# electronicarts/mesh2splat

Hardware: AMD Instinct MI355X
Metric: Gaussians/sec emitted (mesh->3DGS conversion pass, density 1024^2) (higher is better)
Workload: dtype f32

## Files before the change

mesh2splat_amd/csrc/m2s_context.cpp:

```cpp
#include "m2s_ctx.h"

#include <algorithm>
#include <chrono>
#include <cstring>
#include <string>

using namespace m2s;
using namespace m2s_host;

namespace {
thread_local std::string g_create_error = "";
}

namespace m2s_host {
void free_scene(m2s_ctx* c) {
    c->tri_mem.release(); c->scene_arena.release();
    c->lane[0].release_scene(false); c->lane[1].release_scene(true);
    c->d_meshes = nullptr; c->d_mesh_first = nullptr;
    c->d_cnt = c->d_partials = nullptr;
    c->d_biglist = nullptr; c->d_bigmeta = nullptr; c->d_bands = nullptr; c->run_table_words = 0; c->d_run_order = nullptr; c->run_order_unit = 0;
    c->d_batch_first = nullptr; c->n_batch_tab = 0; c->chain_words = 0;
    c->rinfo.clear();
    ++c->rinfo_gen;
    c->frag_per_R2 = -1.0;
    c->warm_R = 0; c->warm_total = 0; c->warm_mismatch_seen = false;
    c->sparse_off_R = c->team_off_R = c->lean_off_R = UINT32_MAX;
    c->lean_ok = false;
    c->d_vt_rows.release(); c->d_vt_ids.release();
    c->vt_rows = 0; c->vt_use = false;
    c->geo_stride = 0; c->geo_use = false;
    c->scene = SceneDev{};
    c->has_scene = false;
}

m2s_ctx::RInfo& rinfo_for(m2s_ctx* c, uint32_t R) {
    auto it = c->rinfo.find(R);
    if (it != c->rinfo.end()) return it->second;
    if (c->rinfo.size() >= (size_t)kBandSlots) { drain_in_flight(c); c->rinfo.clear(); ++c->rinfo_gen; }
    m2s_ctx::RInfo ri;
    ri.gen = c->rinfo_gen;
    ri.band_slot = (int)c->rinfo.size();
    return c->rinfo.emplace(R, ri).first->second;
}

static bool spin_waits() { static const bool on = !debug_on("M2S_NO_SPIN"); return on; }
template <class Query, class Block>
static hipError_t spin_then_block(Query query, Block block) {
    if (spin_waits()) {
        const auto t0 = std::chrono::steady_clock::now();
        for (uint32_t i = 0;; ++i) {
            const hipError_t e = query();
            if (e != hipErrorNotReady) return e;
            if ((i & 15u) == 15u && std::chrono::steady_clock::now() - t0 > std::chrono::microseconds(400)) break;
        }
        (void)hipGetLastError();
    }
    return block();
}
hipError_t wait_stream(hipStream_t st) { return spin_then_block([&] { return hipStreamQuery(st); }, [&] { return hipStreamSynchronize(st); }); }
hipError_t wait_event(hipEvent_t ev) { return spin_then_block([&] { return hipEventQuery(ev); }, [&] { return hipEventSynchronize(ev); }); }

void drain_in_flight(m2s_ctx* c, int lane) {
    each_in_flight(c, [&](m2s_ctx::Slot& sl) {
        if (!sl.sync_result && (lane < 0 || sl.own_lane == lane)) (void)hipEventSynchronize(sl.done[0]);
    });
}

hipError_t next_epoch(m2s_ctx* c, uint32_t* out) {
    const uint32_t e = ++c->epoch;
    *out = e;
    if ((e & 0xFFFFu) != 0) return hipSuccess;
    const size_t bytes = std::max<size_t>(c->chain_words, 1) * sizeof(unsigned long long);
    hipError_t r = hipDeviceSynchronize();
// ... 160 lines not shown
```

mesh2splat_amd/csrc/m2s_ctx.h:

```cpp
#pragma once
#include "../../include/m2s.h"
#include "m2s_devbuf.h"
#include "m2s_device.h"
#include "m2s_recstate.h"
#include "m2s_vdedup.h"

#include <cstdint>
#include <cstdlib>
#include <map>
#include <string>

namespace m2s_host {
constexpr uint32_t kMaxGaussiansToSort = 7000000u;
constexpr uint64_t kMaxTriangles = (1ull << 28) - 1;
inline size_t align_up(size_t v, size_t a) { return (v + a - 1) / a * a; }
inline const char* const kStaleMsg = "the records of the conversion last waited for have been overwritten by a later submission at another R "
                                     "(wait for it, or submit into your own buffers)";
inline const char* const kInFlightMsg = "conversions are still in flight: m2s_convert_wait first";
struct GBufPlanes {
    DevBuf<void> plane[5];
    void* ptr[5] = {};
    m2s_status reserve(std::string& err, uint64_t px) {
        for (int k = 0; k < 5; ++k) {
            const m2s_status s = plane[k].reserve(err, px, (k == 2 || k == 4) ? 4 : 8);
// ... 5 lines not shown
};
}

constexpr int kBandSlotsMax = 64;
struct m2s_ctx : m2s_host::RecordState {
    int device = 0;
    m2s_host::StreamSet<2> streams;
    hipStream_t stream = nullptr;
    std::string err;

    m2s_host::DevBuf<char> tri_mem;
    m2s::SceneDev scene{};
    m2s::MeshParams* d_meshes = nullptr;
    uint32_t* d_mesh_first = nullptr;
    uint32_t n_meshes_total = 0;
    bool has_scene = false;
    bool lean_ok = false;
    uint64_t range_first = 0, range_count = UINT64_MAX;
    m2s_host::DevBuf<float4> d_vt_rows;
    m2s_host::DevBuf<m2s::VtIds> d_vt_ids;
    uint32_t vt_rows = 0;
    bool vt_use = false;
    m2s_host::DevBuf<float4> d_geo;
    size_t geo_stride = 0;
    bool geo_use = false;

    uint32_t* d_cnt = nullptr;
    uint32_t* d_partials = nullptr;
    m2s_host::PinnedBuf<unsigned long long> h_total;
    static constexpr int kPinnedPrepass = 2 + 2 * M2S_MAX_IN_FLIGHT;
    static constexpr int kPinnedSortMM = 4 + 2 * M2S_MAX_IN_FLIGHT;
    static constexpr int kPinnedWords = 6 + 2 * M2S_MAX_IN_FLIGHT;
    m2s::BigItem* d_biglist = nullptr;
    uint32_t* d_bigmeta = nullptr;
    struct RInfo {
        int form = M2S_PIPELINE_AUTO;
        uint32_t tpw = 0;
        bool async_ok = false;
        bool mp_ready = false;
        bool bands_ready = false;
        uint32_t bands_unit = 0;
        int band_slot = 0;
        uint32_t gen = 0;
    };
    uint32_t sparse_off_R = UINT32_MAX, team_off_R = UINT32_MAX, lean_off_R = UINT32_MAX;
    uint32_t rinfo_gen = 0;
    std::map<uint32_t, RInfo> rinfo;
    double frag_per_R2 = -1.0;
    uint64_t warm_total = 0;
    uint64_t warm_big = 0;
    bool warm_mismatch_seen = false;
    uint32_t hint_R = 0;
    uint32_t warm_R = 0;
    int warm_spec_form = 0;
    uint32_t warm_spec_unit = 0, warm_spec_shift = 0;
    unsigned long long* d_bands = nullptr;
    size_t run_table_words = 0;
    uint32_t* d_run_order = nullptr;
    uint32_t run_order_unit = 0, run_order_shift = 0;
    uint32_t* d_batch_first = nullptr;
    uint32_t n_batch_tab = 0;
    size_t chain_words = 0;
    int last_pipeline = 0;
    m2s_host::Lane lane[2];
    int lanes = 1;
    int pipeline = M2S_PIPELINE_AUTO;
    uint32_t epoch = 0;

    struct Slot { m2s_host::EventSet<1> done; m2s_host::EventSet<2> t;
                  uint64_t limit = 0; void* d_out = nullptr; uint32_t R = 0;
                  bool sync_result = false; uint64_t sync_total = 0; bool prof = false; float ms[M2S_K_N] = {};
                  int own_lane = -1; uint32_t gen = 0;
                  bool wrote_bands = false; uint32_t bands_unit = 0; uint32_t ri_gen = 0;
                  hipStream_t st = nullptr; bool shared_work = false; };
    Slot slot[M2S_MAX_IN_FLIGHT];
    uint32_t slot_head = 0, slot_count = 0;

    int64_t cap_policy = -1;

    m2s_host::DevBuf<float4> d_sorted;
    m2s_host::DevBuf<uint32_t> d_sort_u32;
    uint32_t sorted_key_offset = 0;
    m2s_host::DevBuf<void> d_sort_temp;
    float last_sort_ms = 0.0f;
    float last_sort_stage_ms[3] = { 0, 0, 0 };
    m2s_host::ClockOf<m2s_host::SortMark> sort_clock;
    m2s_host::DevBuf<float4> d_pos_plane;
    bool keep_positions = false;
    m2s_host::DevBuf<float4> d_quads;
    m2s_host::DevBuf<float> d_pp_depths;
    m2s_host::DevBuf<unsigned long long> d_pp_chain;
    uint32_t pp_epoch = 0;
    m2s_host::DevBuf<float> d_pp_depthtex;
    float last_prepass_ms = 0.0f;
    m2s_host::ClockOf<m2s_host::SpanMark> prepass_clock;
    m2s_host::PinnedBuf<m2s_gaussian> h_export[2];
    m2s_host::PinnedBuf<char> h_stage[2];
    m2s_host::DevBuf<char> d_stage[2];
    m2s_host::EventSet<2> stage_ev;
    m2s_host::DevBuf<char> scene_arena;
    float last_upload_ms[5] = { 0, 0, 0, 0, 0 };
    m2s_host::DevBuf<uint8_t> d_rows;
    m2s_host::DevBuf<void> d_loaded;
    m2s_host::DevBuf<float4> d_sorted_quads;
    float last_sort_prepass_ms = 0.0f;
    m2s_host::ClockOf<m2s_host::SpanMark> sort_prepass_clock;
    m2s_host::GBufPlanes d_gbuf;
    int32_t gbuf_w = 0, gbuf_h = 0;
    m2s_host::BinWork splat_work;
    m2s_host::DevBuf<uint32_t> d_splat_tiles;
    float last_splat_ms = 0.0f;
    m2s_host::ClockOf<m2s_host::BinMark> bin_clock;
// ... 231 lines not shown
```

mesh2splat_amd/csrc/m2s_device.h:

```cpp
#pragma once
#include <cstdlib>
#include <hip/hip_runtime.h>
#include <stdint.h>

#include "m2s_stageclock.h"
#include "m2s_vtable.h"

namespace m2s {
using m2s_host::StageMarks;

#ifdef M2S_DEBUG_BUILD
inline const char* debug_env(const char* name) {
    static const bool enabled = std::getenv("M2S_DEBUG") != nullptr;
    return enabled ? std::getenv(name) : nullptr;
}
#else
inline const char* debug_env(const char*) { return nullptr; }
#endif
inline bool debug_on(const char* name) { const char* v = debug_env(name); return v && *v && *v != '0'; }

constexpr int kBlock = 256;
constexpr int kTriPerBlock = 1024;
constexpr int kEmitF = 1024;
constexpr int kRowsThread = 32;
// ... 10 lines not shown
    const float4* C1;
    const float*  C2;
    const float4* D0;
    const float4* D1;
    const float4* D2;
};

struct TexDesc {
    const uint32_t* texels;
    uint32_t w, h, n_levels;
    uint32_t off[5];
};

struct ComboDesc {
    const uint32_t* texels;
    uint32_t coff[5];
};

struct MeshParams {
    float bmin[3];
    float bmax[3];
    float color[4];
    TexDesc tex[3];
    ComboDesc combo;
};

struct BigItem {
    uint32_t t, cnt;
    unsigned long long off;
};

struct SceneDev {
    TriPlanes tri;
    const MeshParams* meshes;
    const uint32_t* mesh_first;
    const uint2* mesh_of8;
    uint32_t n_meshes;
    uint32_t n_tri;
    uint32_t tri_first;
};

void launch_repack(const float* d_aos, uint32_t stride_floats, uint32_t n_tri_src, uint32_t src_first,
                   uint32_t n, uint32_t dst_first, TriPlanes dst , hipStream_t st);
void launch_mesh_table(const SceneDev& sc, uint2* table, hipStream_t st);
void launch_mip_level(const uint32_t* src, uint32_t sw, uint32_t sh, uint32_t* dst, uint32_t dw, uint32_t dh,
                      hipStream_t st);
void launch_combo_level(const uint32_t* a, const uint32_t* n, const uint32_t* m, uint32_t w, uint32_t h, uint32_t* dst,
                        hipStream_t st);
void launch_count(const SceneDev& sc, uint32_t R, uint32_t* cnt, uint32_t* partials, hipStream_t st);
void launch_scan_partials(uint32_t* partials, uint32_t n_partials, unsigned long long* total, hipStream_t st);
void launch_big_share(const uint32_t* cnt, uint32_t n_tri, uint32_t threshold, unsigned long long* out, hipStream_t st);
void launch_unit_bases(const uint32_t* cnt, const uint32_t* partials, uint32_t n_tri, uint32_t unit, uint32_t shift, unsigned long long* run_base, hipStream_t st);
void launch_run_order(const unsigned long long* run_base, uint32_t n_runs, const unsigned long long* total, uint32_t* order, uint32_t n_slots,
                      uint32_t first_set, hipStream_t st);
inline uint32_t resident_workgroups(const void* kernel, int threads) {
    int dev = 0, cus = 0, per_cu = 0;
    if (hipGetDevice(&dev) != hipSuccess || hipDeviceGetAttribute(&cus, hipDeviceAttributeMultiprocessorCount, dev) != hipSuccess ||
        hipOccupancyMaxActiveBlocksPerMultiprocessor(&per_cu, kernel, threads, 0) != hipSuccess || cus <= 0 || per_cu <= 0) {
        (void)hipGetLastError();
        return 0u;
    }
    return (uint32_t)per_cu * (uint32_t)cus;
}
uint32_t fused2_resident_workgroups();
uint32_t fused3_resident_workgroups();
uint32_t sparse_resident_workgroups();
inline uint32_t run_order_slots(uint32_t n_units, uint32_t shift) { return ((n_units + (8u << shift) - 1u) / (8u << shift)) * 8u; }
uint32_t emit2_slices(uint64_t limit);
uint32_t count_scan_blocks(uint32_t n_tri);
size_t setup_bytes(uint32_t n_tri);
size_t setup_tall_offset(uint32_t n_tri);
void launch_count_scan(const SceneDev& sc, uint32_t R, uint32_t* off, uint32_t* start, uint32_t n_start, unsigned long long* chain,
                       uint32_t epoch, unsigned long long* total, void* setup, uint32_t* status, unsigned long long* total_host, hipStream_t st);
void launch_emit2(const SceneDev& sc, uint32_t R, const uint32_t* off, const uint32_t* start, const unsigned long long* total,
                  uint64_t limit, const void* setup, float4* out, hipStream_t st);

void launch_encode_rows(const float4* rec, uint64_t n, uint32_t format, float scale_multiplier, uint8_t* out, hipStream_t st);

struct RunInfo {
    const unsigned long long* base;
    unsigned long long* out;
    uint32_t shift;
    const uint32_t* order;
};
inline uint32_t run_shift_for(uint32_t n_units) {
    if (const char* v = debug_env("M2S_RUN_SHIFT")) { const uint32_t s = (uint32_t)std::atoi(v) & 15u; return n_units >= (32u << s) ? s : 0u; }
    for (uint32_t shift = 5; shift >= 3; --shift)
        if (n_units >= (32u << shift)) return shift;
    return 0u;
}
inline uint32_t n_runs(uint32_t n_units, uint32_t shift) { return (n_units + (1u << shift) - 1u) >> shift; }
struct BatchTable {
    const uint32_t* first;
    uint32_t n;
    uint32_t tpw;
};
uint32_t fused2_band_workgroups(uint32_t n_tri);
void launch_fused2(const SceneDev& sc, uint32_t R, unsigned long long* chain, uint64_t limit, float4* out,
                   unsigned long long* total, uint32_t* status, uint32_t epoch, BigItem* biglist, uint32_t* bigmeta,
                   const RunInfo& runs, const BatchTable& batches, hipStream_t st);
struct GeoPlanes {
    const float4* G0;
    const float4* G1;
    const float4* G2;
};
void launch_geo_planes(const SceneDev& sc, float4* g0, float4* g1, float4* g2, hipStream_t st);
void launch_fused3(const SceneDev& sc, uint32_t R, unsigned long long* chain, uint64_t limit, float4* out,
                   unsigned long long* total, uint32_t* status, uint32_t epoch, BigItem* biglist, uint32_t* bigmeta,
                   const RunInfo& runs, const BatchTable& batches, hipStream_t st, const VtxTable* vt = nullptr,
                   const GeoPlanes* gp = nullptr);
void launch_sparse(const SceneDev& sc, uint32_t R, unsigned long long* chain, uint64_t limit, float4* out,
                   unsigned long long* total, uint32_t* status, uint32_t epoch, BigItem* biglist, uint32_t* bigmeta,
                   const RunInfo& runs, hipStream_t st, float4* plane = nullptr);
bool sparse_supported(uint32_t n_tri);
uint32_t sparse_workgroups(uint32_t n_tri);
constexpr uint32_t kSparseTrianglesPerWorkgroup = 512;
void launch_emit_big(const SceneDev& sc, uint32_t R, const BigItem* biglist, uint32_t n_big, uint32_t max_cnt, uint64_t limit,
                     float4* out, hipStream_t st);

struct PrepassK {
// ... 233 lines not shown
```

mesh2splat_amd/csrc/m2s_kernels.hip:

```cpp
#include "m2s_devfn.h"

#pragma clang fp contract(off)

namespace m2s {

struct TriPlanesW {
    float4* A0; float4* A1; float* A2; float4* B0; float2* B1; float4* C0; float4* C1; float* C2;
    float4* D0; float4* D1; float4* D2;
};

__global__ void __launch_bounds__(kBlock) k_repack(const float* __restrict__ aos, uint32_t stride, uint32_t src_first,
                                                   uint32_t n, uint32_t dst_first, TriPlanesW d) {
    uint32_t i = blockIdx.x * kBlock + threadIdx.x;
    if (i >= n) return;
    const float* v0 = aos + (size_t)(src_first + i) * 3 * stride;
    const float* v1 = v0 + stride;
    const float* v2 = v1 + stride;
    uint32_t t = dst_first + i;
    d.A0[t] = make_float4(v0[0], v0[1], v0[2], v1[0]);
    d.A1[t] = make_float4(v1[1], v1[2], v2[0], v2[1]);
    d.A2[t] = v2[2];
    d.B0[t] = make_float4(v0[10], v0[11], v1[10], v1[11]);
    d.B1[t] = make_float2(v2[10], v2[11]);
    d.C0[t] = make_float4(v0[3], v0[4], v0[5], v1[3]);
    d.C1[t] = make_float4(v1[4], v1[5], v2[3], v2[4]);
    d.C2[t] = v2[5];
    d.D0[t] = make_float4(v0[6], v0[7], v0[8], v0[9]);
    d.D1[t] = make_float4(v1[6], v1[7], v1[8], v1[9]);
    d.D2[t] = make_float4(v2[6], v2[7], v2[8], v2[9]);
}

void launch_repack(const float* d_aos, uint32_t stride_floats, uint32_t , uint32_t src_first, uint32_t n,
                   uint32_t dst_first, TriPlanes dst, hipStream_t st) {
    if (!n) return;
    TriPlanesW w;
    w.A0 = const_cast<float4*>(dst.A0); w.A1 = const_cast<float4*>(dst.A1); w.A2 = const_cast<float*>(dst.A2);
    w.B0 = const_cast<float4*>(dst.B0); w.B1 = const_cast<float2*>(dst.B1);
    w.C0 = const_cast<float4*>(dst.C0); w.C1 = const_cast<float4*>(dst.C1); w.C2 = const_cast<float*>(dst.C2);
    w.D0 = const_cast<float4*>(dst.D0); w.D1 = const_cast<float4*>(dst.D1); w.D2 = const_cast<float4*>(dst.D2);
    hipLaunchKernelGGL(k_repack, dim3((n + kBlock - 1) / kBlock), dim3(kBlock), 0, st, d_aos, stride_floats, src_first, n,
                       dst_first, w);
}

__global__ void __launch_bounds__(kBlock) k_mip(const uint32_t* __restrict__ src, uint32_t sw, uint32_t sh,
                                                uint32_t* __restrict__ dst, uint32_t dw, uint32_t dh) {
    uint32_t i = blockIdx.x * kBlock + threadIdx.x;
    if (i >= dw * dh) return;
    uint32_t x = i % dw, y = i / dw;
    uint32_t x0 = min(2 * x, sw - 1), x1 = min(2 * x + 1, sw - 1);
    uint32_t y0 = min(2 * y, sh - 1), y1 = min(2 * y + 1, sh - 1);
    uint32_t t00 = src[(size_t)y0 * sw + x0], t10 = src[(size_t)y0 * sw + x1];
    uint32_t t01 = src[(size_t)y1 * sw + x0], t11 = src[(size_t)y1 * sw + x1];
    uint32_t o = 0;
// ... 117 lines not shown
        if (threadIdx.x == 1023) carry_s = carry + woff + incl;
        __syncthreads();
    }
    if (threadIdx.x == 0) *total = carry_s;
}

void launch_scan_partials(uint32_t* partials, uint32_t n_partials, unsigned long long* total, hipStream_t st) {
    hipLaunchKernelGGL(k_scan_partials, dim3(1), dim3(1024), 0, st, partials, n_partials, total);
}

__global__ void __launch_bounds__(kBlock) k_big_share(const uint32_t* __restrict__ cnt, uint32_t n, uint32_t threshold, unsigned long long* __restrict__ out) {
    unsigned long long acc = 0;
    for (uint32_t i = blockIdx.x * kBlock + threadIdx.x; i < n; i += gridDim.x * kBlock) {
        const uint32_t c = cnt[i];
        if (c > threshold) acc += c;
    }
#pragma unroll
    for (int d = 32; d >= 1; d >>= 1) acc += __shfl_xor(acc, d);
    if ((threadIdx.x & 63) == 0 && acc) atomicAdd(out, acc);
}
void launch_big_share(const uint32_t* cnt, uint32_t n_tri, uint32_t threshold, unsigned long long* out, hipStream_t st) {
    if (!n_tri) return;
    hipLaunchKernelGGL(k_big_share, dim3(std::min<uint32_t>((n_tri + kBlock - 1) / kBlock, 1024u)), dim3(kBlock), 0, st, cnt, n_tri, threshold, out);
}

__global__ void __launch_bounds__(kBlock) k_unit_bases(const uint32_t* __restrict__ cnt, const uint32_t* __restrict__ partials,
                                                       uint32_t n_tri, uint32_t unit, uint32_t shift, unsigned long long* __restrict__ run_base) {
    __shared__ uint32_t red[kTriPerBlock / kBlock][kBlock / 64];
    const int lane = threadIdx.x & 63, wave = threadIdx.x >> 6;
    const uint32_t blockBase = blockIdx.x * kTriPerBlock;
#pragma unroll
    for (int it = 0; it < kTriPerBlock / kBlock; ++it) {
        const uint32_t t = blockBase + it * kBlock + threadIdx.x;
        const uint32_t s = wave_sum(t < n_tri ? cnt[t] : 0u);
        if (lane == 0) red[it][wave] = s;
    }
    __syncthreads();
    if (threadIdx.x == 0) {
        unsigned long long run = partials[blockIdx.x];
        const uint32_t tri_per_run = unit << shift;
        for (int it = 0; it < kTriPerBlock / kBlock; ++it) {
            const uint32_t t = blockBase + it * kBlock;
            if (t < n_tri && t % tri_per_run == 0) run_base[t / tri_per_run] = run;
            run += red[it][0] + red[it][1] + red[it][2] + red[it][3];
        }
    }
}

void launch_unit_bases(const uint32_t* cnt, const uint32_t* partials, uint32_t n_tri, uint32_t unit, uint32_t shift, unsigned long long* run_base, hipStream_t st) {
    if (!n_tri) return;
    hipLaunchKernelGGL(k_unit_bases, dim3(n_count_blocks(n_tri)), dim3(kBlock), 0, st, cnt, partials, n_tri, unit, shift, run_base);
}

__device__ __forceinline__ uint32_t run_order_slot_of_rank(uint32_t rank, uint32_t n_runs, uint32_t first_set) {
    const uint32_t groups = (first_set < n_runs ? first_set : n_runs) / 8u;
    if (groups < 2u) return rank;
    const uint32_t heavy = ((groups + 1u) / 2u) * 8u, light = (groups / 2u) * 8u;
    if (rank < heavy) return rank;
    if (rank >= n_runs - light) {
        const uint32_t j = n_runs - 1u - rank;
        return (groups - 1u - (j >> 3)) * 8u + (j & 7u);
    }
    return rank + light;
}
__global__ void __launch_bounds__(kBlock) k_run_order(const unsigned long long* __restrict__ run_base, uint32_t n_runs,
                                                      const unsigned long long* __restrict__ total, uint32_t* __restrict__ order, uint32_t n_slots,
                                                      uint32_t first_set) {
    const uint32_t i = blockIdx.x * kBlock + threadIdx.x;
    if (i >= n_slots) return;
    if (i >= n_runs) { order[i] = i; return; }
    const unsigned long long end = *total;
    auto cost = [&](uint32_t j) { return (j + 1u < n_runs ? run_base[j + 1u] : end) - run_base[j]; };
    const unsigned long long mine = cost(i);
    uint32_t rank = 0;
    for (uint32_t j = 0; j < n_runs; ++j) {
        const unsigned long long cj = cost(j);
        rank += (cj > mine || (cj == mine && j < i)) ? 1u : 0u;
    }
    order[run_order_slot_of_rank(rank, n_runs, first_set)] = i;
}
void launch_run_order(const unsigned long long* run_base, uint32_t n_runs, const unsigned long long* total, uint32_t* order, uint32_t n_slots,
                      uint32_t first_set, hipStream_t st) {
    if (!n_slots) return;
    hipLaunchKernelGGL(k_run_order, dim3((n_slots + kBlock - 1) / kBlock), dim3(kBlock), 0, st, run_base, n_runs, total, order, n_slots, first_set);
}

__global__ void __launch_bounds__(kBlock) k_emit_big(SceneDev sc, uint32_t R, const BigItem* __restrict__ list, uint32_t n_big,
                                                     unsigned long long limit, float4* __restrict__ out) {
    __shared__ uint2 entries[kEmitF];
    __shared__ float4 stage[kBlock * kStageStride];
    __shared__ uint32_t rowoff[4096 + 1];
    __shared__ uint16_t rowxa[4096];
    __shared__ uint32_t wsum[kBlock / 64];
    if (blockIdx.y >= n_big) return;
    const BigItem item = list[blockIdx.y];
    const uint32_t f0 = blockIdx.x * kEmitF;
    if (f0 >= item.cnt) return;
    const uint32_t f1 = min(f0 + (uint32_t)kEmitF, item.cnt);
    if (item.off + f0 >= limit) return;
    const int lane = threadIdx.x & 63, wave = threadIdx.x >> 6;
    const uint32_t m = find_mesh(sc, sc.tri_first + item.t);
    Raster rs;
    if (!setup_raster_for(sc, item.t, m, true, R, rs)) return;
    const int rows = rs.y1 - rs.y0 + 1;
    uint32_t local[16], tsum = 0;
#pragma unroll
    for (int k = 0; k < 16; ++k) {
        const int r = threadIdx.x * 16 + k;
        uint32_t len = 0;
        if (r < rows) {
            int xa, xb;
            row_span(rs, rs.y0 + r, xa, xb);
            len = (uint32_t)max(xb - xa + 1, 0);
            rowxa[r] = (uint16_t)xa;
        }
        local[k] = len;
        tsum += len;
    }
    const uint32_t incl = wave_incl_scan(tsum, lane);
    if (lane == 63) wsum[wave] = incl;
    __syncthreads();
    uint32_t run = incl - tsum;
    for (int w = 0; w < wave; ++w) run += wsum[w];
#pragma unroll
    for (int k = 0; k < 16; ++k) {
        const int r = threadIdx.x * 16 + k;
        if (r < rows) rowoff[r] = run;
        run += local[k];
    }
    if (threadIdx.x == kBlock - 1) rowoff[rows] = run;
    __syncthreads();
    for (uint32_t f = f0 + threadIdx.x; f < f1; f += kBlock) {
        int lo = 0, hi = rows;
        while (hi - lo > 1) {
            const int mid = (lo + hi) >> 1;
            if (rowoff[mid] <= f) lo = mid; else hi = mid;
        }
// ... 51 lines not shown
```

mesh2splat_amd/csrc/m2s_pass.cpp:

```cpp
#include "m2s_ctx.h"

#include <algorithm>
#include <cstdio>
#include <cstring>
#include <vector>

using namespace m2s;
using namespace m2s_host;

namespace {
static double sparse_frags_per_triangle(uint32_t n_tri) { return n_tri >= 2000000u ? 1.75 : 0.5; }
static uint32_t band_workgroups(const m2s_ctx* c, uint32_t unit) {
    const uint32_t team = fused2_band_workgroups(c->scene.n_tri);
    return !team ? 0u : unit == 256u ? team : sparse_workgroups(c->scene.n_tri);
}
static uint32_t first_resident_slots([[maybe_unused]] int form, [[maybe_unused]] uint32_t shift) {
#ifdef M2S_RUN_ORDER_SPREAD
    const uint32_t wgs = form == M2S_PIPELINE_SPARSE ? sparse_resident_workgroups() : form == M2S_PIPELINE_LEAN ? fused3_resident_workgroups()
                                                                                                                 : fused2_resident_workgroups();
    return wgs >> shift;
#else
    return 0u;
#endif
}
}

namespace m2s_host {
RunInfo bands_for(const m2s_ctx* c, const m2s_ctx::RInfo& ri, uint32_t unit, bool may_write, bool* writes) {
    RunInfo r{ nullptr, nullptr, 0u, nullptr };
    if (writes) *writes = false;
    const uint32_t n_wg = band_workgroups(c, unit);
    const uint32_t shift = run_shift_for(n_wg);
    if (!n_wg || !shift || !c->d_bands || !c->run_table_words || (unit == 256u && (c->n_batch_tab || ri.tpw)) || debug_on("M2S_NO_BANDS")) return r;
    if ((size_t)n_runs(n_wg, shift) > c->run_table_words) return r;
    unsigned long long* table = c->d_bands + (size_t)ri.band_slot * c->run_table_words;
    r.shift = shift;
    if (ri.bands_ready && ri.bands_unit == unit) {
        r.base = table;
        if (c->run_order_unit == unit && c->run_order_shift == shift && !debug_on("M2S_NO_RUN_ORDER")) r.order = c->d_run_order;
    }
    else if (may_write) { r.out = table; if (writes) *writes = true; }
    return r;
}

BatchTable batches_for(const m2s_ctx* c, const m2s_ctx::RInfo& ri) {
    return c->n_batch_tab ? BatchTable{ c->d_batch_first, c->n_batch_tab, 0u } : BatchTable{ nullptr, 0u, ri.tpw };
}

uint32_t unit_of(int form) { return form == M2S_PIPELINE_SPARSE ? kSparseTrianglesPerWorkgroup : 256u; }

void launch_single(const m2s_ctx* c, const m2s_ctx::RInfo& ri, uint32_t R, unsigned long long* chain, uint64_t limit, float4* d_out,
                   unsigned long long* res, uint32_t epoch, const RunInfo& runs, hipStream_t st, float4* plane) {
    uint32_t* status = reinterpret_cast<uint32_t*>(&res[1]);
    if (ri.form == M2S_PIPELINE_SPARSE)
        launch_sparse(c->scene, R, chain, limit, d_out, &res[0], status, epoch, c->d_biglist, c->d_bigmeta, runs, st, plane);
    else if (ri.form == M2S_PIPELINE_LEAN) {
        const VtxTable vt{ c->d_vt_rows.get(), c->d_vt_ids.get() };
        const GeoPlanes gp{ c->d_geo.get(), c->d_geo.get() + c->geo_stride, c->d_geo.get() + 2 * c->geo_stride };
        launch_fused3(c->scene, R, chain, limit, d_out, &res[0], status, epoch, c->d_biglist, c->d_bigmeta, runs, batches_for(c, ri), st,
                      c->vt_use ? &vt : nullptr, c->geo_use ? &gp : nullptr);
    }
    else
        launch_fused2(c->scene, R, chain, limit, d_out, &res[0], status, epoch, c->d_biglist, c->d_bigmeta, runs, batches_for(c, ri), st);
}

uint64_t resolve_cap(const m2s_ctx* c, uint32_t R) {
    if (c->cap_policy == 0) return 0;
    if (c->cap_policy > 0) return (uint64_t)c->cap_policy;
    const uint32_t mc = std::max<uint32_t>(1u, c->n_meshes_total);
    const uint32_t mx = R * R * 6u * mc;
    return std::min(mx, kMaxGaussiansToSort);
}
}

static bool lean_eligible(const m2s_ctx* c, uint32_t R) {
    if (!c->lean_ok || R >= c->lean_off_R || debug_on("M2S_NO_LEAN")) return false;
// ... 6 lines not shown
    ri.form = M2S_PIPELINE_MULTIPASS;
    if (c->pipeline == M2S_PIPELINE_MULTIPASS || R >= c->team_off_R) return;
    if (c->pipeline == M2S_PIPELINE_AUTO && frags >= 11.0 * n_tri) {
        if (frags < 13.0 * n_tri && R == c->warm_R && c->warm_total > 0 && c->warm_big * 8ull < c->warm_total &&
            fused_tpw(c->scene.n_tri) == 64u && !c->n_batch_tab && !debug_on("M2S_NO_BAND_TPW")) {
            ri.form = M2S_PIPELINE_TEAM;
            ri.tpw = 40;
        }
        return;
    }
    const bool sparse = c->pipeline == M2S_PIPELINE_SPARSE ||
                        (c->pipeline == M2S_PIPELINE_AUTO && frags < sparse_frags_per_triangle(c->scene.n_tri) * n_tri && !debug_on("M2S_NO_SPARSE"));
    if (sparse && R < c->sparse_off_R && sparse_supported(c->scene.n_tri)) ri.form = M2S_PIPELINE_SPARSE;
    else ri.form = lean_eligible(c, R) ? M2S_PIPELINE_LEAN : M2S_PIPELINE_TEAM;
}

enum class Trouble { full, stalled, lean_defers, big_share };

static void demote(m2s_ctx* c, m2s_ctx::RInfo& ri, uint32_t R, Trouble why) {
    const bool every_larger_R = why == Trouble::full || why == Trouble::lean_defers;
    if (why == Trouble::big_share) {
        ri.form = M2S_PIPELINE_MULTIPASS;
    } else if (ri.form == M2S_PIPELINE_SPARSE) {
        if (every_larger_R) c->sparse_off_R = std::min(c->sparse_off_R, R);
        ri.form = lean_eligible(c, R) ? M2S_PIPELINE_LEAN : M2S_PIPELINE_TEAM;
    } else if (ri.form == M2S_PIPELINE_LEAN) {
        if (every_larger_R) c->lean_off_R = std::min(c->lean_off_R, R);
        ri.form = M2S_PIPELINE_TEAM;
    } else {
        if (ri.tpw) ri.tpw = 0;
        else if (every_larger_R) c->team_off_R = std::min(c->team_off_R, R);
        ri.form = M2S_PIPELINE_MULTIPASS;
    }
}

namespace m2s_host {
m2s_status warm_count_enqueue(m2s_ctx* c, uint32_t R) {
    const SceneDev& sc = c->scene;
    if (!sc.n_tri || R == 0 || R > 4096) return M2S_ERR_INVALID;
    hipStream_t st = c->stream;
    launch_count(sc, R, c->d_cnt, c->d_partials, st);
    launch_scan_partials(c->d_partials, n_count_blocks(sc.n_tri), c->lane[0].total, st);
    HIPCHK(c, hipGetLastError());
    HIPCHK(c, hipMemcpyAsync(c->h_total, c->lane[0].total, 8, hipMemcpyDeviceToHost, st));
    c->warm_spec_unit = 0;
    if (!debug_on("M2S_NO_WARM_BANDS")) {
        m2s_ctx::RInfo& ri = rinfo_for(c, R);
        const uint32_t unit = unit_of(M2S_PIPELINE_TEAM);
        bool writes = false;
        const RunInfo table = bands_for(c, ri, unit, true, &writes);
        if (writes) {
            const uint32_t n_units = band_workgroups(c, unit);
            launch_unit_bases(c->d_cnt, c->d_partials, sc.n_tri, unit, table.shift, table.out, st);
            const int form = lean_eligible(c, R) ? M2S_PIPELINE_LEAN : M2S_PIPELINE_TEAM;
            launch_run_order(table.out, n_runs(n_units, table.shift), c->lane[0].total, c->d_run_order, run_order_slots(n_units, table.shift),
                             first_resident_slots(form, table.shift), st);
            HIPCHK(c, hipGetLastError());
            c->warm_spec_unit = unit; c->warm_spec_shift = table.shift; c->warm_spec_form = form;
        }
    }
    return M2S_OK;
}

m2s_status warm_scene(m2s_ctx* c, uint32_t R, bool counted) {
    const SceneDev& sc = c->scene;
    if (!sc.n_tri || R == 0 || R > 4096) return M2S_OK;
    hipStream_t st = c->stream;
    if (!counted) {
        const m2s_status s = warm_count_enqueue(c, R);
        if (s != M2S_OK) return s;
        HIPCHK(c, hipStreamSynchronize(st));
    }
    const uint64_t total = c->h_total[0];
    c->frag_per_R2 = (double)total / ((double)R * (double)R);
    c->warm_R = R;
    c->warm_total = total;
    c->warm_big = 0;
    if (total >= 11ull * sc.n_tri && total < 13ull * sc.n_tri) {
        HIPCHK(c, hipMemsetAsync(c->lane[0].total, 0, 8, st));
        launch_big_share(c->d_cnt, sc.n_tri, 96u, c->lane[0].total, st);
        HIPCHK(c, hipGetLastError());
        HIPCHK(c, hipMemcpyAsync(&c->h_total[1], c->lane[0].total, 8, hipMemcpyDeviceToHost, st));
        HIPCHK(c, hipStreamSynchronize(st));
        c->warm_big = c->h_total[1];
        c->h_total[1] = 0;
        const unsigned long long tot = total;
        HIPCHK(c, hipMemcpy(c->lane[0].total, &tot, sizeof tot, hipMemcpyHostToDevice));
    }
    if (batch_table_capacity(sc.n_tri) && !c->n_batch_tab && !debug_on("M2S_NO_BATCH_TABLE")) {
        try {
            std::vector<uint32_t> cnt(sc.n_tri), first;
            HIPCHK(c, hipMemcpy(cnt.data(), c->d_cnt, (size_t)sc.n_tri * sizeof(uint32_t), hipMemcpyDeviceToHost));
            uint32_t n_target = n_fused_waves(sc.n_tri);
            if (const char* v = debug_env("M2S_BATCH_TARGET")) { const unsigned long q = strtoul(v, nullptr, 10); if (q >= 1 && q <= 8192) n_target = (uint32_t)q; }
            double ct = 214.0;
            const double cf = 140.0;
            if (const char* v = debug_env("M2S_BATCH_CT")) ct = atof(v);
            double total = 0.0;
            for (uint32_t t = 0; t < sc.n_tri; ++t) total += ct + cf * (double)cnt[t];
            const double quota = total / (double)n_target;
            first.reserve(batch_table_capacity(sc.n_tri));
            first.push_back(0);
            double acc = 0.0;
            uint32_t in_batch = 0;
            for (uint32_t g = 0; g < sc.n_tri; g += 8) {
                const uint32_t ge = std::min(g + 8u, sc.n_tri);
                double gc = 0.0;
                for (uint32_t t = g; t < ge; ++t) gc += ct + cf * (double)cnt[t];
                if (in_batch && (in_batch + (ge - g) > 64u || acc + 0.5 * gc >= quota * (double)first.size())) { first.push_back(g); in_batch = 0; }
                acc += gc;
                in_batch += ge - g;
            }
            first.push_back(sc.n_tri);
            if (first.size() <= batch_table_capacity(sc.n_tri)) {
                HIPCHK(c, hipMemcpy(c->d_batch_first, first.data(), first.size() * sizeof(uint32_t), hipMemcpyHostToDevice));
                c->n_batch_tab = (uint32_t)first.size() - 1u;
            }
        } catch (...) {  }
    }
    m2s_ctx::RInfo& ri = rinfo_for(c, R);
    if (ri.form == M2S_PIPELINE_AUTO) decide(c, ri, (double)total, R);
    const uint64_t cap = resolve_cap(c, R);
    const bool single = ri.form != M2S_PIPELINE_MULTIPASS;
    if (!debug_on("M2S_NO_PRELOAD")) {
        if (!single) { (void)preload_multipass(); if (!debug_on("M2S_NO_SCRATCH_WARM")) launch_scratch_warm(st); }
        else if (ri.form == M2S_PIPELINE_SPARSE) { (void)preload_sparse(); (void)preload_fused2(); }
        else if (ri.form == M2S_PIPELINE_LEAN) { (void)preload_fused3(); }
        else { (void)preload_fused2(); }
        (void)hipGetLastError();
    }
    if (single && !debug_on("M2S_NO_WARM_BANDS")) {
        const uint32_t unit = unit_of(ri.form);
        bool writes = false;
        const RunInfo table = bands_for(c, ri, unit, true, &writes);
        if (writes) {
            const bool spec_order = c->warm_spec_form == ri.form || first_resident_slots(ri.form, table.shift) == 0u;
            if (!(counted && c->warm_spec_unit == unit && c->warm_spec_shift == table.shift && spec_order)) {
                launch_unit_bases(c->d_cnt, c->d_partials, sc.n_tri, unit, table.shift, table.out, st);
                const uint32_t n_units = band_workgroups(c, unit);
                launch_run_order(table.out, n_runs(n_units, table.shift), c->lane[0].total, c->d_run_order, run_order_slots(n_units, table.shift),
                                 first_resident_slots(ri.form, table.shift), st);
                HIPCHK(c, hipGetLastError());
                HIPCHK(c, hipStreamSynchronize(st));
            }
            c->run_order_unit = unit; c->run_order_shift = table.shift;
            ri.bands_ready = true; ri.bands_unit = unit;
        }
    }
    const uint64_t want = cap ? cap : std::max<uint64_t>(total, 1);
    if (c->hint_R != 0 || c->lane[0].records) {
        if (!single || total >= 8ull * sc.n_tri) (void)ensure_lane(c, 0, true, emit2_slices(std::min<uint64_t>(cap ? cap : want, 0xFFFFFFFFull)));
        (void)ensure_records(c, want);
    }
    c->err.clear();
    return M2S_OK;
}
}


namespace m2s_host {
m2s_status ensure_lane(m2s_ctx* c, int L, bool multipass, uint32_t n_start) {
    Lane& ln = c->lane[L];
    const Lane& l0 = c->lane[0];
    const uint32_t n_tri = c->scene.n_tri;
    bool fresh = false;
    if (L) {
        M2S_TRY(c->streams.ensure(c->err, L));
        ln.stream = c->streams[L];
        const size_t words = std::max<size_t>(c->chain_words, 1);
        M2S_TRY(ln.chain_own.reserve(c->err, words, sizeof(unsigned long long), &fresh));
        ln.chain = ln.chain_own;
        if (fresh) HIPCHK(c, hipMemsetAsync(ln.chain, 0, words * sizeof(unsigned long long), ln.stream));
        if (ln.records.cap() < l0.records.cap()) {
            drain_in_flight(c, L);
            M2S_TRY(ln.records.reserve(c->err, l0.records.cap(), sizeof(m2s_gaussian)));
            ++ln.rec_gen;
        }
    }
    if (!multipass) return M2S_OK;
    if (L) {
        M2S_TRY(ln.off_own.reserve(c->err, std::max<size_t>(n_tri, 1) + 1, sizeof(uint32_t)));
        ln.off = ln.off_own;
    }
    uint64_t slices = ln.start.cap();
    if (slices < n_start) {
        drain_in_flight(c, L ? L : -1);
        slices = std::max<uint64_t>(std::max<uint64_t>(n_start, 2 * slices), std::max<uint64_t>(l0.start.cap(), 16384));
    }
    M2S_TRY(ln.reserve_work(c->err, slices, setup_bytes(n_tri), &fresh));
    if (fresh) {
        HIPCHK(c, hipMemsetAsync((char*)ln.setup.get() + setup_tall_offset(n_tri), 0, 16, ln.stream));
        HIPCHK(c, hipStreamSynchronize(ln.stream));
    }
    return M2S_OK;
// ... 190 lines not shown
```

mesh2splat_amd/csrc/m2s_upload.cpp:

```cpp
#include "m2s_ctx.h"
#include "m2s_ply.h"

#include <algorithm>
#include <array>
#include <chrono>
#include <cstring>
#include <thread>
#include <tuple>
#include <vector>

using namespace m2s;
using namespace m2s_host;

namespace {
constexpr size_t kStageChunk = 16ull << 20;

void par_memcpy(void* dst, const void* src, size_t n) {
    const size_t kMin = 2ull << 20;
    unsigned nt = (unsigned)std::min<size_t>(4, n / kMin);
    if (const char* e = std::getenv("M2S_HOST_THREADS")) { if (std::atol(e) == 1) nt = 1; }
    if (nt <= 1) { memcpy(dst, src, n); return; }
    std::vector<std::thread> pool;
    for (unsigned i = 1; i < nt; ++i) {
        const size_t b = n * i / nt, e = n * (i + 1) / nt;
// ... 97 lines not shown
            auto it = dedup.find(key);
            if (it != dedup.end()) { mesh_tex[i][k] = (int)it->second; continue; }
            TexPlan p{};
            p.src = t.rgba8;
            p.d.w = t.width; p.d.h = t.height;
            uint32_t mx = std::max(t.width, t.height), nl = 1;
            while (mx > 1 && nl < 5) { mx >>= 1; nl++; }
            p.d.n_levels = nl;
            size_t tot = 0;
            for (uint32_t l = 0; l < nl; ++l) {
                p.d.off[l] = (uint32_t)tot;
                tot += (size_t)std::max(1u, t.width >> l) * std::max(1u, t.height >> l);
            }
            p.arena_off = take(tot * 4);
            dedup[key] = (uint32_t)tex_plan.size();
            mesh_tex[i][k] = (int)tex_plan.size();
            tex_plan.push_back(p);
        }
        const int ia = mesh_tex[i][0], in = mesh_tex[i][1], im = mesh_tex[i][2];
        if (ia < 0 || in < 0 || im < 0) continue;
        const TexDesc &ta = tex_plan[ia].d, &tn = tex_plan[in].d, &tm = tex_plan[im].d;
        if (ta.w != tn.w || ta.w != tm.w || ta.h != tn.h || ta.h != tm.h) continue;
        const auto ckey = std::make_tuple((uint32_t)ia, (uint32_t)in, (uint32_t)im);
        auto cit = cdedup.find(ckey);
        if (cit != cdedup.end()) { mesh_combo[i] = (int)cit->second; continue; }
        ComboPlan cp{};
        size_t tot = 0;
        for (uint32_t l = 0; l < ta.n_levels; ++l) {
            cp.d.coff[l] = (uint32_t)tot;
            tot += (size_t)(std::max(1u, ta.w >> l) + 1) * std::max(1u, ta.h >> l) * 3;
        }
        if (tot > 0x3FFFFFF0ull) continue;
        cp.arena_off = take(tot * 4);
        cp.ia = (uint32_t)ia; cp.in = (uint32_t)in; cp.im = (uint32_t)im;
        cdedup[ckey] = (uint32_t)combo_plan.size();
        mesh_combo[i] = (int)combo_plan.size();
        combo_plan.push_back(cp);
    }
    const size_t n_mp = std::max<uint32_t>(n_meshes, 1);
    const size_t chain_words = std::max<size_t>(std::max<size_t>(std::max<size_t>(n_fused_waves(n_tri), batch_table_capacity(n_tri)), (size_t)n_tri / 32 + 1), 1);
    const size_t o_meshes = take(n_mp * sizeof(MeshParams));
    const size_t o_mesh_first = take(mesh_first.size() * sizeof(uint32_t));
    const size_t o_mesh_of8 = take(((np + 7) / 8 + 1) * sizeof(uint2));
    const size_t o_cnt = take(np * sizeof(uint32_t));
    const size_t o_off = take((np + 1) * sizeof(uint32_t));
    const size_t o_partials = take(std::max<size_t>(n_count_blocks(n_tri), 1) * sizeof(uint32_t));
    const size_t o_chain = take(chain_words * sizeof(unsigned long long));
    const size_t o_biglist = take(np * sizeof(BigItem));
    const size_t o_bigmeta = take(4 * sizeof(uint32_t));
    const uint32_t units = fused2_band_workgroups(n_tri);
    const size_t run_words = run_shift_for(units) ? (size_t)n_runs(units, run_shift_for(units)) + 1 : 0;
    const size_t o_bands = take(std::max<size_t>((size_t)kBandSlots * run_words, 1) * sizeof(unsigned long long));
    const size_t o_run_order = take(std::max<size_t>(run_shift_for(units) ? run_order_slots(units, run_shift_for(units)) : 0, 1) * sizeof(uint32_t));
    const size_t o_batch = take(std::max<size_t>(batch_table_capacity(n_tri), 1) * sizeof(uint32_t));
    M2S_TRY(c->scene_arena.reserve(c->err, arena, 1));
    M2S_TRY(ensure_stage(c));
    c->last_upload_ms[3] = ms_since(t_alloc);
    char* A = c->scene_arena;
    char* b = c->tri_mem;
    TriPlanes& tp = c->scene.tri;
    tp.A0 = (const float4*)(b + offs[0]); tp.A1 = (const float4*)(b + offs[1]); tp.A2 = (const float*)(b + offs[2]);
    tp.B0 = (const float4*)(b + offs[3]); tp.B1 = (const float2*)(b + offs[4]);
    tp.C0 = (const float4*)(b + offs[5]); tp.C1 = (const float4*)(b + offs[6]); tp.C2 = (const float*)(b + offs[7]);
    tp.D0 = (const float4*)(b + offs[8]); tp.D1 = (const float4*)(b + offs[9]); tp.D2 = (const float4*)(b + offs[10]);

    const auto t_geo = std::chrono::steady_clock::now();
    uint32_t turn = 0;
    for (uint32_t i = 0; i < n_meshes && n_tri; ++i) {
        const uint64_t s = std::max<uint64_t>(first, mesh_first[i]), e = std::min<uint64_t>(last, mesh_first[i + 1]);
        if (e <= s) continue;
        const uint32_t stride = meshes[i].stride_floats;
        const size_t tri_bytes = (size_t)3 * stride * sizeof(float);
        const size_t per_chunk = std::max<size_t>(1, kStageChunk / tri_bytes) * tri_bytes;
        const char* src = (const char*)(meshes[i].vertices + (size_t)(s - mesh_first[i]) * 3 * stride);
        const uint32_t dst0 = (uint32_t)(s - first);
        const m2s_status st = staged_h2d(c, src, (size_t)(e - s) * tri_bytes, per_chunk, nullptr, turn,
            [&](char* d, size_t off, size_t n) {
                launch_repack((const float*)d, stride, (uint32_t)(n / tri_bytes), 0, (uint32_t)(n / tri_bytes),
                              dst0 + (uint32_t)(off / tri_bytes), tp, c->stream);
            });
        if (st != M2S_OK) return st;
    }
    c->last_upload_ms[1] = ms_since(t_geo);

    const auto t_tex = std::chrono::steady_clock::now();
    for (TexPlan& p : tex_plan) p.d.texels = (uint32_t*)(A + p.arena_off);
    for (ComboPlan& cp : combo_plan) cp.d.texels = (uint32_t*)(A + cp.arena_off);
    std::vector<MeshParams> mp(n_mp);
    memset(mp.data(), 0, mp.size() * sizeof(MeshParams));
    for (uint32_t i = 0; i < n_meshes; ++i) {
        const m2s_mesh& m = meshes[i];
        MeshParams& p = mp[i];
        memcpy(p.bmin, m.bbox_min, 12);
        memcpy(p.bmax, m.bbox_max, 12);
        memcpy(p.color, m.base_color, 16);
        for (int k = 0; k < 3; ++k) if (mesh_tex[i][k] >= 0) p.tex[k] = tex_plan[mesh_tex[i][k]].d;
        if (mesh_combo[i] >= 0) p.combo = combo_plan[mesh_combo[i]].d;
    }
    c->lean_ok = true;
    for (uint32_t i = 0; i < n_meshes; ++i)
        if (mesh_combo[i] < 0 && (mesh_tex[i][0] >= 0 || mesh_tex[i][1] >= 0 || mesh_tex[i][2] >= 0)) c->lean_ok = false;
    c->d_meshes = (MeshParams*)(A + o_meshes);
    c->d_mesh_first = (uint32_t*)(A + o_mesh_first);
    HIPCHK(c, hipMemcpyAsync(c->d_meshes, mp.data(), mp.size() * sizeof(MeshParams), hipMemcpyHostToDevice, c->stream));
    HIPCHK(c, hipMemcpyAsync(c->d_mesh_first, mesh_first.data(), mesh_first.size() * sizeof(uint32_t), hipMemcpyHostToDevice, c->stream));
    c->scene.meshes = c->d_meshes;
    c->scene.mesh_first = c->d_mesh_first;
    c->scene.mesh_of8 = (const uint2*)(A + o_mesh_of8);
    launch_mesh_table(c->scene, (uint2*)(A + o_mesh_of8), c->stream);

    c->d_cnt = (uint32_t*)(A + o_cnt);
    c->lane[0].off = (uint32_t*)(A + o_off);
    c->d_partials = (uint32_t*)(A + o_partials);
    c->lane[0].chain = (unsigned long long*)(A + o_chain);
    c->d_biglist = (BigItem*)(A + o_biglist);
    c->d_bigmeta = (uint32_t*)(A + o_bigmeta);
    c->d_bands = (unsigned long long*)(A + o_bands);
    c->run_table_words = run_words;
    c->d_run_order = (uint32_t*)(A + o_run_order);
    c->run_order_unit = 0; c->run_order_shift = 0;
    c->d_batch_first = (uint32_t*)(A + o_batch);
    c->n_batch_tab = 0;
    c->chain_words = chain_words;
    HIPCHK(c, hipMemsetAsync(c->lane[0].chain, 0, chain_words * sizeof(unsigned long long), c->stream));
    HIPCHK(c, hipMemsetAsync(c->d_bigmeta, 0, 4 * sizeof(uint32_t), c->stream));
    const uint32_t warm_R = c->hint_R ? c->hint_R : converted_R(c) ? converted_R(c) : 1024u;
    const bool warm = !debug_on("M2S_NO_WARM");
    bool counted = false;
    if (warm && !debug_on("M2S_NO_WARM_OVERLAP")) counted = warm_count_enqueue(c, warm_R) == M2S_OK;
    VtWork vt_work;
    bool vt_begun = false;
    if (vt_size_ok(c->lean_ok, n_tri) && !debug_on("M2S_NO_VTABLE")) {
        vt_begun = vt_dedup_begin(tp, n_tri, vt_work, c->stream) == hipSuccess;
        if (!vt_begun) (void)hipGetLastError();
    }
    if (vt_size_ok(c->lean_ok, n_tri) && !debug_on("M2S_NO_GEOPLANES")) {
        const size_t stride = align_up((size_t)n_tri * sizeof(float4), 256) / sizeof(float4);
        if (c->d_geo.try_reserve(3 * stride, sizeof(float4))) {
            launch_geo_planes(c->scene, c->d_geo.get(), c->d_geo.get() + stride, c->d_geo.get() + 2 * stride, c->stream);
            c->geo_stride = stride;
            c->geo_use = true;
        }
    }
    if (!c->geo_use) c->d_geo.release();

    for (TexPlan& p : tex_plan) {
        uint32_t* mem = (uint32_t*)(A + p.arena_off);
        const m2s_status st = staged_h2d(c, (const char*)p.src, (size_t)p.d.w * p.d.h * 4, kStageChunk, (char*)mem, turn,
                                         [](char*, size_t, size_t) {});
        if (st != M2S_OK) return st;
        for (uint32_t l = 1; l < p.d.n_levels; ++l)
            launch_mip_level(mem + p.d.off[l - 1], std::max(1u, p.d.w >> (l - 1)), std::max(1u, p.d.h >> (l - 1)),
                             mem + p.d.off[l], std::max(1u, p.d.w >> l), std::max(1u, p.d.h >> l), c->stream);
    }
    for (ComboPlan& cp : combo_plan) {
        uint32_t* mem = (uint32_t*)(A + cp.arena_off);
        const TexDesc &ta = tex_plan[cp.ia].d, &tn = tex_plan[cp.in].d, &tm = tex_plan[cp.im].d;
        for (uint32_t l = 0; l < ta.n_levels; ++l)
            launch_combo_level(ta.texels + ta.off[l], tn.texels + tn.off[l], tm.texels + tm.off[l], std::max(1u, ta.w >> l),
                               std::max(1u, ta.h >> l), mem + cp.d.coff[l], c->stream);
    }
    HIPCHK(c, hipStreamSynchronize(c->stream));
    HIPCHK(c, hipGetLastError());
    if (vt_begun) {
        if (vt_dedup_finish(tp, n_tri, vt_work, kVtIdLimit, kVtMinSharing, c->d_vt_rows, c->d_vt_ids, &c->vt_rows, &c->vt_use, c->stream) != hipSuccess) {
            (void)hipGetLastError();
            c->d_vt_rows.release(); c->d_vt_ids.release();
            c->vt_use = false;
        }
    }
    c->last_upload_ms[2] = ms_since(t_tex);
    c->has_scene = true;
// ... 41 lines not shown
```

Baseline: 29.76 billion.

## Balance run order across eight queues with greedy least-loaded assignment

Replaces the fixed rank-to-slot interleave, which only applied a heavy/light split when a compile flag was set, with two kernels. The first ranks runs by cost, and a single-thread kernel then greedily places each run on the least-loaded of eight queues. It adds a scratch buffer in the scene arena and drops the warm-spec form bookkeeping. The goal is more even work across the persistent workgroups that consume runs, at the cost of an extra launch and a serial assignment loop on one thread.

```diff
diff --git a/mesh2splat_amd/csrc/m2s_context.cpp b/mesh2splat_amd/csrc/m2s_context.cpp
--- a/mesh2splat_amd/csrc/m2s_context.cpp
+++ b/mesh2splat_amd/csrc/m2s_context.cpp
@@ -18,7 +18,7 @@
     c->lane[0].release_scene(false); c->lane[1].release_scene(true);
     c->d_meshes = nullptr; c->d_mesh_first = nullptr;
     c->d_cnt = c->d_partials = nullptr;
-    c->d_biglist = nullptr; c->d_bigmeta = nullptr; c->d_bands = nullptr; c->run_table_words = 0; c->d_run_order = nullptr; c->run_order_unit = 0;
+    c->d_biglist = nullptr; c->d_bigmeta = nullptr; c->d_bands = nullptr; c->run_table_words = 0; c->d_run_order = nullptr; c->d_run_rank = nullptr; c->run_order_unit = 0;
     c->d_batch_first = nullptr; c->n_batch_tab = 0; c->chain_words = 0;
     c->rinfo.clear();
     ++c->rinfo_gen;
diff --git a/mesh2splat_amd/csrc/m2s_ctx.h b/mesh2splat_amd/csrc/m2s_ctx.h
--- a/mesh2splat_amd/csrc/m2s_ctx.h
+++ b/mesh2splat_amd/csrc/m2s_ctx.h
@@ -81,12 +81,12 @@
     bool warm_mismatch_seen = false;
     uint32_t hint_R = 0;
     uint32_t warm_R = 0;
-    int warm_spec_form = 0;
     uint32_t warm_spec_unit = 0, warm_spec_shift = 0;
     unsigned long long* d_bands = nullptr;
     size_t run_table_words = 0;
     uint32_t* d_run_order = nullptr;
     uint32_t run_order_unit = 0, run_order_shift = 0;
+    void* d_run_rank = nullptr;
     uint32_t* d_batch_first = nullptr;
     uint32_t n_batch_tab = 0;
     size_t chain_words = 0;
diff --git a/mesh2splat_amd/csrc/m2s_device.h b/mesh2splat_amd/csrc/m2s_device.h
--- a/mesh2splat_amd/csrc/m2s_device.h
+++ b/mesh2splat_amd/csrc/m2s_device.h
@@ -86,7 +86,7 @@
 void launch_big_share(const uint32_t* cnt, uint32_t n_tri, uint32_t threshold, unsigned long long* out, hipStream_t st);
 void launch_unit_bases(const uint32_t* cnt, const uint32_t* partials, uint32_t n_tri, uint32_t unit, uint32_t shift, unsigned long long* run_base, hipStream_t st);
 void launch_run_order(const unsigned long long* run_base, uint32_t n_runs, const unsigned long long* total, uint32_t* order, uint32_t n_slots,
-                      uint32_t first_set, hipStream_t st);
+                      void* scratch, hipStream_t st);
 inline uint32_t resident_workgroups(const void* kernel, int threads) {
     int dev = 0, cus = 0, per_cu = 0;
     if (hipGetDevice(&dev) != hipSuccess || hipDeviceGetAttribute(&cus, hipDeviceAttributeMultiprocessorCount, dev) != hipSuccess ||
@@ -100,6 +100,7 @@
 uint32_t fused3_resident_workgroups();
 uint32_t sparse_resident_workgroups();
 inline uint32_t run_order_slots(uint32_t n_units, uint32_t shift) { return ((n_units + (8u << shift) - 1u) / (8u << shift)) * 8u; }
+inline size_t run_order_scratch_bytes(uint32_t n_slots) { return (size_t)n_slots * (sizeof(unsigned long long) + sizeof(uint32_t)); }
 uint32_t emit2_slices(uint64_t limit);
 uint32_t count_scan_blocks(uint32_t n_tri);
 size_t setup_bytes(uint32_t n_tri);
diff --git a/mesh2splat_amd/csrc/m2s_kernels.hip b/mesh2splat_amd/csrc/m2s_kernels.hip
--- a/mesh2splat_amd/csrc/m2s_kernels.hip
+++ b/mesh2splat_amd/csrc/m2s_kernels.hip
@@ -1,4 +1,5 @@
 #include "m2s_devfn.h"
+#include "m2s_run_balance.h"
 
 #pragma clang fp contract(off)
 
@@ -222,23 +223,11 @@
     hipLaunchKernelGGL(k_unit_bases, dim3(n_count_blocks(n_tri)), dim3(kBlock), 0, st, cnt, partials, n_tri, unit, shift, run_base);
 }
 
-__device__ __forceinline__ uint32_t run_order_slot_of_rank(uint32_t rank, uint32_t n_runs, uint32_t first_set) {
-    const uint32_t groups = (first_set < n_runs ? first_set : n_runs) / 8u;
-    if (groups < 2u) return rank;
-    const uint32_t heavy = ((groups + 1u) / 2u) * 8u, light = (groups / 2u) * 8u;
-    if (rank < heavy) return rank;
-    if (rank >= n_runs - light) {
-        const uint32_t j = n_runs - 1u - rank;
-        return (groups - 1u - (j >> 3)) * 8u + (j & 7u);
-    }
-    return rank + light;
-}
-__global__ void __launch_bounds__(kBlock) k_run_order(const unsigned long long* __restrict__ run_base, uint32_t n_runs,
-                                                      const unsigned long long* __restrict__ total, uint32_t* __restrict__ order, uint32_t n_slots,
-                                                      uint32_t first_set) {
+__global__ void __launch_bounds__(kBlock) k_run_rank(const unsigned long long* __restrict__ run_base, uint32_t n_runs,
+                                                     const unsigned long long* __restrict__ total, unsigned long long* __restrict__ cost_by_rank,
+                                                     uint32_t* __restrict__ run_by_rank) {
     const uint32_t i = blockIdx.x * kBlock + threadIdx.x;
-    if (i >= n_slots) return;
-    if (i >= n_runs) { order[i] = i; return; }
+    if (i >= n_runs) return;
     const unsigned long long end = *total;
     auto cost = [&](uint32_t j) { return (j + 1u < n_runs ? run_base[j + 1u] : end) - run_base[j]; };
     const unsigned long long mine = cost(i);
@@ -247,12 +236,22 @@
         const unsigned long long cj = cost(j);
         rank += (cj > mine || (cj == mine && j < i)) ? 1u : 0u;
     }
-    order[run_order_slot_of_rank(rank, n_runs, first_set)] = i;
+    cost_by_rank[rank] = mine;
+    run_by_rank[rank] = i;
+}
+__global__ void __launch_bounds__(kBlock) k_run_assign(const unsigned long long* __restrict__ cost_by_rank, const uint32_t* __restrict__ run_by_rank,
+                                                       uint32_t n_runs, uint32_t n_slots, uint32_t* order) {
+    if (threadIdx.x == 0) run_balance_assign(cost_by_rank, n_runs, n_slots, order);
+    __syncthreads();
+    for (uint32_t s = threadIdx.x; s < n_runs; s += kBlock) order[s] = run_by_rank[order[s]];
 }
 void launch_run_order(const unsigned long long* run_base, uint32_t n_runs, const unsigned long long* total, uint32_t* order, uint32_t n_slots,
-                      uint32_t first_set, hipStream_t st) {
-    if (!n_slots) return;
-    hipLaunchKernelGGL(k_run_order, dim3((n_slots + kBlock - 1) / kBlock), dim3(kBlock), 0, st, run_base, n_runs, total, order, n_slots, first_set);
+                      void* scratch, hipStream_t st) {
+    if (!n_slots || !n_runs || n_runs > n_slots) return;
+    unsigned long long* cost_by_rank = static_cast<unsigned long long*>(scratch);
+    uint32_t* run_by_rank = reinterpret_cast<uint32_t*>(cost_by_rank + n_slots);
+    hipLaunchKernelGGL(k_run_rank, dim3((n_runs + kBlock - 1) / kBlock), dim3(kBlock), 0, st, run_base, n_runs, total, cost_by_rank, run_by_rank);
+    hipLaunchKernelGGL(k_run_assign, dim3(1), dim3(kBlock), 0, st, cost_by_rank, run_by_rank, n_runs, n_slots, order);
 }
 
 __global__ void __launch_bounds__(kBlock) k_emit_big(SceneDev sc, uint32_t R, const BigItem* __restrict__ list, uint32_t n_big,
diff --git a/mesh2splat_amd/csrc/m2s_pass.cpp b/mesh2splat_amd/csrc/m2s_pass.cpp
--- a/mesh2splat_amd/csrc/m2s_pass.cpp
+++ b/mesh2splat_amd/csrc/m2s_pass.cpp
@@ -13,15 +13,6 @@
 static uint32_t band_workgroups(const m2s_ctx* c, uint32_t unit) {
     const uint32_t team = fused2_band_workgroups(c->scene.n_tri);
     return !team ? 0u : unit == 256u ? team : sparse_workgroups(c->scene.n_tri);
-}
-static uint32_t first_resident_slots([[maybe_unused]] int form, [[maybe_unused]] uint32_t shift) {
-#ifdef M2S_RUN_ORDER_SPREAD
-    const uint32_t wgs = form == M2S_PIPELINE_SPARSE ? sparse_resident_workgroups() : form == M2S_PIPELINE_LEAN ? fused3_resident_workgroups()
-                                                                                                                 : fused2_resident_workgroups();
-    return wgs >> shift;
-#else
-    return 0u;
-#endif
 }
 }
 
@@ -134,11 +125,10 @@
         if (writes) {
             const uint32_t n_units = band_workgroups(c, unit);
             launch_unit_bases(c->d_cnt, c->d_partials, sc.n_tri, unit, table.shift, table.out, st);
-            const int form = lean_eligible(c, R) ? M2S_PIPELINE_LEAN : M2S_PIPELINE_TEAM;
             launch_run_order(table.out, n_runs(n_units, table.shift), c->lane[0].total, c->d_run_order, run_order_slots(n_units, table.shift),
-                             first_resident_slots(form, table.shift), st);
+                             c->d_run_rank, st);
             HIPCHK(c, hipGetLastError());
-            c->warm_spec_unit = unit; c->warm_spec_shift = table.shift; c->warm_spec_form = form;
+            c->warm_spec_unit = unit; c->warm_spec_shift = table.shift;
         }
     }
     return M2S_OK;
@@ -216,12 +206,11 @@
         bool writes = false;
         const RunInfo table = bands_for(c, ri, unit, true, &writes);
         if (writes) {
-            const bool spec_order = c->warm_spec_form == ri.form || first_resident_slots(ri.form, table.shift) == 0u;
-            if (!(counted && c->warm_spec_unit == unit && c->warm_spec_shift == table.shift && spec_order)) {
+            if (!(counted && c->warm_spec_unit == unit && c->warm_spec_shift == table.shift)) {
                 launch_unit_bases(c->d_cnt, c->d_partials, sc.n_tri, unit, table.shift, table.out, st);
                 const uint32_t n_units = band_workgroups(c, unit);
                 launch_run_order(table.out, n_runs(n_units, table.shift), c->lane[0].total, c->d_run_order, run_order_slots(n_units, table.shift),
-                                 first_resident_slots(ri.form, table.shift), st);
+                                 c->d_run_rank, st);
                 HIPCHK(c, hipGetLastError());
                 HIPCHK(c, hipStreamSynchronize(st));
             }
diff --git a/mesh2splat_amd/csrc/m2s_run_balance.h b/mesh2splat_amd/csrc/m2s_run_balance.h
--- /dev/null
+++ b/mesh2splat_amd/csrc/m2s_run_balance.h
@@ -0,0 +1,40 @@
+#pragma once
+#include <cstdint>
+
+#if defined(__HIPCC__) || defined(__CUDACC__)
+#define M2S_RB_HD __host__ __device__
+#else
+#define M2S_RB_HD
+#endif
+
+namespace m2s {
+constexpr uint32_t kRunQueues = 8;
+
+M2S_RB_HD inline void run_balance_assign(const unsigned long long* cost, uint32_t n_runs, uint32_t n_slots, uint32_t* order) {
+    unsigned long long load[kRunQueues];
+    uint32_t used[kRunQueues], cap[kRunQueues];
+    for (uint32_t x = 0; x < kRunQueues; ++x) {
+        load[x] = 0ull;
+        used[x] = 0u;
+        cap[x] = n_runs > x ? (n_runs - x + kRunQueues - 1u) / kRunQueues : 0u;
+    }
+    for (uint32_t i = n_runs; i < n_slots; ++i) order[i] = i;
+    for (uint32_t r = 0; r < n_runs; ++r) {
+        const unsigned long long c = cost[r];
+        uint32_t best = kRunQueues, best_used = 0u;
+        unsigned long long best_load = 0ull;
+        for (uint32_t k = 0; k < kRunQueues; ++k) {
+            const uint32_t x = kRunQueues - 1u - k;
+            const bool free_slot = used[x] < cap[x];
+            const bool better = best == kRunQueues || load[x] < best_load || (load[x] == best_load && used[x] < best_used);
+            if (free_slot && better) { best = x; best_load = load[x]; best_used = used[x]; }
+        }
+        order[best_used * kRunQueues + best] = r;
+        for (uint32_t x = 0; x < kRunQueues; ++x) {
+            const bool hit = x == best;
+            load[x] += hit ? c : 0ull;
+            used[x] += hit ? 1u : 0u;
+        }
+    }
+}
+}
diff --git a/mesh2splat_amd/csrc/m2s_upload.cpp b/mesh2splat_amd/csrc/m2s_upload.cpp
--- a/mesh2splat_amd/csrc/m2s_upload.cpp
+++ b/mesh2splat_amd/csrc/m2s_upload.cpp
@@ -173,6 +173,7 @@
     const size_t run_words = run_shift_for(units) ? (size_t)n_runs(units, run_shift_for(units)) + 1 : 0;
     const size_t o_bands = take(std::max<size_t>((size_t)kBandSlots * run_words, 1) * sizeof(unsigned long long));
     const size_t o_run_order = take(std::max<size_t>(run_shift_for(units) ? run_order_slots(units, run_shift_for(units)) : 0, 1) * sizeof(uint32_t));
+    const size_t o_run_rank = take(run_order_scratch_bytes(run_shift_for(units) ? run_order_slots(units, run_shift_for(units)) : 0));
     const size_t o_batch = take(std::max<size_t>(batch_table_capacity(n_tri), 1) * sizeof(uint32_t));
     M2S_TRY(c->scene_arena.reserve(c->err, arena, 1));
     M2S_TRY(ensure_stage(c));
@@ -239,6 +240,7 @@
     c->d_bands = (unsigned long long*)(A + o_bands);
     c->run_table_words = run_words;
     c->d_run_order = (uint32_t*)(A + o_run_order);
+    c->d_run_rank = A + o_run_rank;
     c->run_order_unit = 0; c->run_order_shift = 0;
     c->d_batch_first = (uint32_t*)(A + o_batch);
     c->n_batch_tab = 0;
```

Result: faster. 30.26 billion, median of 6 (+1.7%).
